# Infini-AI-Lab/Sequoia

Measured on NVIDIA H100. Metric: decoded tokens/sec (mean accepted len/step in config.accepted_tokens_per_step), Sequoia tree speculative decoding, 68m->7B Llama (config c2 unless --config says otherwise), higher is better.
Workload: dtype f16

## Files before the change

sequoia_b200/csrc/sq_gemm.cu:

```cuda
#include <cstdio>
#include <cstdlib>

#include "sq_common.cuh"
#include "sq_ptx.cuh"

struct sq_gemm_plan {
  CUtensorMap tm_a, tm_w;
  __half* c;
  int ldc, n_max, N, K, bn, split, stages, mc, pdl, tiled, epi, n_out;
  int* err_flag;
};

namespace sq {

struct GemmArgs {
  __half* c;
  int ldc, n, N, K, kb_per_split;
  int tiled, kb_total;
  int m0;
  int epi, n_out;
  int* err_flag;
};

constexpr int G_BK = 64;
constexpr int G_THREADS = 384;
constexpr int G_CONSUMER_WARPS = 8;

template <int BN, int STAGES, int SPLIT>
struct GemmSmem {
  static constexpr int A_BYTES = 128 * 128;
  static constexpr int W_BYTES = BN * 128;
  static constexpr int STAGE_BYTES = A_BYTES + ((W_BYTES + 1023) / 1024) * 1024;
  static constexpr int OFF_BAR = STAGES * STAGE_BYTES;
  static constexpr int OFF_RED = OFF_BAR + 256;
  static constexpr int R_STRIDE = BN + 4;
  static constexpr int RED_BYTES = SPLIT > 1 ? 128 * R_STRIDE * 4 : 0;
  static constexpr int TOTAL = OFF_RED + RED_BYTES;
};

__device__ __forceinline__ void tma_load_2d_mc(uint32_t dst, const CUtensorMap* tm, uint32_t bar, int c0, int c1, uint16_t mask) {
  asm volatile(
      "cp.async.bulk.tensor.2d.shared::cluster.global.mbarrier::complete_tx::bytes.multicast::cluster [%0], [%1, {%4, %5}], [%2], %3;" ::"r"(dst),
      "l"(tm), "r"(bar), "h"(mask), "r"(c0), "r"(c1)
      : "memory");
}

template <int BN, int STAGES, int SPLIT, int MC>
__global__ void __launch_bounds__(G_THREADS, 1)
    gemm_tn_kernel(const __grid_constant__ CUtensorMap tm_a, const __grid_constant__ CUtensorMap tm_w, GemmArgs g) {
  using SM = GemmSmem<BN, STAGES, SPLIT>;
  constexpr int NCH = BN / 64;
  extern __shared__ __align__(1024) uint8_t smem_raw[];
  uint8_t* smem = smem_raw + ((1024u - (ptx::smem_u32(smem_raw) & 1023u)) & 1023u);
  const int tid = threadIdx.x, warp = tid >> 5, lane = tid & 31;
  const int n0 = blockIdx.x * BN;
  const int ks = blockIdx.y;
  const int mcr = (MC > 1) ? (int)(blockIdx.x % MC) : 0;
  const int kb0 = ks * g.kb_per_split;
  const int nkb = g.kb_per_split;
  const uint32_t s_base = ptx::smem_u32(smem);
  const uint32_t bar_full = s_base + SM::OFF_BAR, bar_empty = bar_full + 8 * STAGES;

  if (tid == 0) {
#pragma unroll
    for (int s = 0; s < STAGES; ++s) {
      ptx::mbar_init(bar_full + 8 * s, 1);
      ptx::mbar_init(bar_empty + 8 * s, G_CONSUMER_WARPS * MC);
    }
    ptx::fence_barrier_init();
  }
  __syncthreads();
  if (MC > 1)
    asm volatile("barrier.cluster.arrive.release.aligned;\n\tbarrier.cluster.wait.acquire.aligned;" ::: "memory");

  if (warp < 4) {
    if (tid == 0) {
      asm volatile("griddepcontrol.launch_dependents;" ::: "memory");
      const int pre = nkb < STAGES ? nkb : STAGES;
      for (int kb = 0; kb < pre; ++kb) {
        const uint32_t sa = s_base + kb * SM::STAGE_BYTES, sw = sa + SM::A_BYTES;
        ptx::mbar_expect_tx(bar_full + 8 * kb, SM::A_BYTES + SM::W_BYTES);
        if (g.tiled) ptx::tma_load_2d(sw, &tm_w, bar_full + 8 * kb, 0, ((int)blockIdx.x * g.kb_total + kb0 + kb) * BN);
        else ptx::tma_load_2d(sw, &tm_w, bar_full + 8 * kb, (kb0 + kb) * G_BK, n0);
      }
      asm volatile("griddepcontrol.wait;" ::: "memory");
      int stage = 0;
      uint32_t phase = 0;
      for (int kb = 0; kb < nkb; ++kb) {
        const uint32_t sa = s_base + stage * SM::STAGE_BYTES, sw = sa + SM::A_BYTES;
        if (kb >= pre) {
          ptx::mbar_wait_one(bar_empty + 8 * stage, phase ^ 1, g.err_flag, 11);
          ptx::mbar_expect_tx(bar_full + 8 * stage, SM::A_BYTES + SM::W_BYTES);
          if (g.tiled) ptx::tma_load_2d(sw, &tm_w, bar_full + 8 * stage, 0, ((int)blockIdx.x * g.kb_total + kb0 + kb) * BN);
          else ptx::tma_load_2d(sw, &tm_w, bar_full + 8 * stage, (kb0 + kb) * G_BK, n0);
        }
        if (MC == 1) ptx::tma_load_2d(sa, &tm_a, bar_full + 8 * stage, (kb0 + kb) * G_BK, g.m0);
        else tma_load_2d_mc(sa + mcr * (SM::A_BYTES / MC), &tm_a, bar_full + 8 * stage, (kb0 + kb) * G_BK, g.m0 + mcr * (128 / MC),
                            (uint16_t)(((1u << MC) - 1u) << (MC * ks)));
        if (++stage == STAGES) { stage = 0; phase ^= 1; }
      }
    }
  } else {
    const int wg = (warp >> 2) - 1;
    float acc[NCH][32];
#pragma unroll
    for (int c = 0; c < NCH; ++c)
#pragma unroll
      for (int e = 0; e < 32; ++e) acc[c][e] = 0.f;
    auto release = [&](int s) {
      if (lane == 0) {
        if (MC == 1) asm volatile("mbarrier.arrive.shared::cta.b64 _, [%0];" ::"r"(bar_empty + 8 * s) : "memory");
        else
          for (int r = 0; r < MC; ++r) ptx::mbar_arrive_cluster(bar_empty + 8 * s, (uint32_t)(MC * ks + r));
      }
    };
    int stage = 0, prev = -1;
    uint32_t phase = 0;
    for (int kb = 0; kb < nkb; ++kb) {
      ptx::mbar_wait(bar_full + 8 * stage, phase, g.err_flag, 12);
      const uint32_t sa = s_base + stage * SM::STAGE_BYTES + wg * 8192, sw = s_base + stage * SM::STAGE_BYTES + SM::A_BYTES;
      ptx::wgmma_fence();
#pragma unroll
      for (int k = 0; k < G_BK / 16; ++k)
#pragma unroll
        for (int c = 0; c < NCH; ++c)
          ptx::wgmma_ss<0>(acc[c], gmma_desc(sa + k * 32, 16, 1024), gmma_desc(sw + c * 8192 + k * 32, 16, 1024), 1);
      ptx::wgmma_commit();
      asm volatile("wgmma.wait_group.sync.aligned 1;" ::: "memory");
      if (prev >= 0) release(prev);
      prev = stage;
      if (++stage == STAGES) { stage = 0; phase ^= 1; }
    }
    ptx::wgmma_wait_all();
    if (prev >= 0) release(prev);
    const int rbase = wg * 64 + (warp & 3) * 16 + (lane >> 2), q2 = 2 * (lane & 3);
    if (SPLIT == 1 && g.epi == 1) {
#pragma unroll
      for (int h = 0; h < 2; ++h) {
        const int row = rbase + 8 * h;
        if (row >= g.n) continue;
        __half* orow = g.c + (int64_t)(g.m0 + row) * g.ldc;
#pragma unroll
        for (int c = 0; c < NCH; ++c)
#pragma unroll
          for (int j = 0; j < 8; ++j) {
            if ((j & 3) >= 2) continue;
            const int ob = (n0 + c * 64 + (j >> 2) * 32) / 2;
            if (ob >= g.n_out) continue;
            __half o[2];
#pragma unroll
            for (int e = 0; e < 2; ++e) {
              const float x = h2f(f2h(acc[c][4 * j + 2 * h + e]));
              const __half act = f2h(x / (1.0f + expf(-x)));
              o[e] = f2h(h2f(act) * h2f(f2h(acc[c][4 * (j + 2) + 2 * h + e])));
            }
            *reinterpret_cast<__half2*>(orow + ob + (j & 3) * 8 + q2) = __halves2half2(o[0], o[1]);
          }
      }
    } else if (SPLIT == 1) {
#pragma unroll
      for (int h = 0; h < 2; ++h) {
        const int row = rbase + 8 * h;
        if (row >= g.n) continue;
        __half* crow = g.c + (int64_t)(g.m0 + row) * g.ldc + n0;
#pragma unroll
        for (int c = 0; c < NCH; ++c)
#pragma unroll
          for (int j = 0; j < 8; ++j)
            if (n0 + c * 64 + j * 8 < g.N)
              *reinterpret_cast<__half2*>(crow + c * 64 + j * 8 + q2) =
                  __floats2half2_rn(acc[c][4 * j + 2 * h], acc[c][4 * j + 2 * h + 1]);
      }
    } else {
      constexpr int RPC = 128 / SPLIT;
#pragma unroll
      for (int h = 0; h < 2; ++h) {
        const int row = rbase + 8 * h;
        uint32_t dst;
        asm volatile("mapa.shared::cluster.u32 %0, %1, %2;" : "=r"(dst) : "r"(s_base + SM::OFF_RED), "r"((uint32_t)mcr + MC * (row / RPC)));
        dst += (uint32_t)((ks * RPC + row % RPC) * SM::R_STRIDE * 4);
#pragma unroll
        for (int c = 0; c < NCH; ++c)
#pragma unroll
          for (int j = 0; j < 8; ++j)
            asm volatile("st.shared::cluster.v2.f32 [%0], {%1, %2};" ::"r"(dst + (c * 64 + j * 8 + q2) * 4),
                         "f"(acc[c][4 * j + 2 * h]), "f"(acc[c][4 * j + 2 * h + 1])
                         : "memory");
      }
    }
  }
  __syncthreads();

  if (MC > 1 || SPLIT > 1)
    asm volatile("barrier.cluster.arrive.release.aligned;\n\tbarrier.cluster.wait.acquire.aligned;" ::: "memory");

  if (SPLIT > 1) {
    constexpr int RPC = 128 / SPLIT;
    constexpr int CPR = BN / 4;
    const float* red = reinterpret_cast<const float*>(smem + SM::OFF_RED);
    for (int i = tid; i < RPC * CPR; i += G_THREADS) {
      const int lr = i / CPR, cc = i % CPR;
      const int row = ks * RPC + lr;
      if (row >= g.n) continue;
      float4 acc = make_float4(0.f, 0.f, 0.f, 0.f);
#pragma unroll
      for (int s = 0; s < SPLIT; ++s) {
        const float4 o = *reinterpret_cast<const float4*>(red + (s * RPC + lr) * SM::R_STRIDE + cc * 4);
        acc.x += o.x; acc.y += o.y; acc.z += o.z; acc.w += o.w;
      }
      const __half2 lo = __floats2half2_rn(acc.x, acc.y), hi = __floats2half2_rn(acc.z, acc.w);
      uint2 pk;
      pk.x = *reinterpret_cast<const uint32_t*>(&lo);
      pk.y = *reinterpret_cast<const uint32_t*>(&hi);
      *reinterpret_cast<uint2*>(g.c + (int64_t)(g.m0 + row) * g.ldc + n0 + cc * 4) = pk;
    }
  }
}

}

using namespace sq;

typedef CUresult (*PFN_tmapEncodeTiledG)(CUtensorMap*, CUtensorMapDataType, cuuint32_t, void*, const cuuint64_t*,
                                         const cuuint64_t*, const cuuint32_t*, const cuuint32_t*, CUtensorMapInterleave,
                                         CUtensorMapSwizzle, CUtensorMapL2promotion, CUtensorMapFloatOOBfill);

static int encode_2d(CUtensorMap* tm, const void* base, uint64_t inner, uint64_t outer, uint64_t pitch_bytes,
                     uint32_t box_inner, uint32_t box_outer, CUtensorMapL2promotion prom) {
  static PFN_tmapEncodeTiledG fn = nullptr;
  if (!fn) {
    void* p = nullptr;
    cudaDriverEntryPointQueryResult qres;
    if (cudaGetDriverEntryPoint("cuTensorMapEncodeTiled", &p, cudaEnableDefault, &qres) == cudaSuccess &&
        qres == cudaDriverEntryPointSuccess)
      fn = (PFN_tmapEncodeTiledG)p;
  }
  if (!fn) { set_error("cuTensorMapEncodeTiled unavailable"); return SQ_ERR_CUDA; }
  cuuint64_t dims[2] = {inner, outer};
  cuuint64_t strides[1] = {pitch_bytes};
  cuuint32_t box[2] = {box_inner, box_outer};
  cuuint32_t estr[2] = {1, 1};
  CUresult r = fn(tm, CU_TENSOR_MAP_DATA_TYPE_FLOAT16, 2, const_cast<void*>(base), dims, strides, box, estr,
                  CU_TENSOR_MAP_INTERLEAVE_NONE, CU_TENSOR_MAP_SWIZZLE_128B, prom, CU_TENSOR_MAP_FLOAT_OOB_FILL_NONE);
  if (r != CUDA_SUCCESS) { set_error("cuTensorMapEncodeTiled failed: %d", (int)r); return SQ_ERR_CUDA; }
  return SQ_OK;
}

static int sm_count() {
  static int n_sm = 0;
  if (!n_sm) {
    int dev = 0;
    if (cudaGetDevice(&dev) != cudaSuccess || cudaDeviceGetAttribute(&n_sm, cudaDevAttrMultiProcessorCount, dev) != cudaSuccess ||
        n_sm <= 0) {
      cudaGetLastError();
      n_sm = 132;
    }
  }
  return n_sm;
}

static void choose_tiles(sq_gemm_plan* p, bool allow_split) {
  const int N = p->N, kb = p->K / 64;
  const int n_sm = sm_count();
  const int cands[] = {256, 192, 128, 64};
  int best_bn = 128, best_split = 1, best_mc = 1;
  double best_score = -1.0;
  for (int bn : cands) {
    const int tiles = (N + bn - 1) / bn;
    for (int split : {1, 2, 4}) {
      if (kb % split || (split > 1 && !allow_split)) continue;
      if (split > 1 && (bn > 128 || N % bn)) continue;
      const int ctas = tiles * split;
      if (ctas > n_sm) continue;
      for (int mc : {1, 2}) {
        if (mc == 2 && tiles % 2) continue;
        const double a_share = 128.0 / mc, share = bn / (bn + a_share);
        double score = ctas * share;
        if (split > 1) score *= 0.85;
        if (score > best_score) { best_score = score; best_bn = bn; best_split = split; best_mc = mc; }
      }
    }
  }
  p->bn = best_bn; p->split = best_split; p->mc = best_mc;
}

static void pick_tiles(sq_gemm_plan* p) {
  const int kb = p->K / 64;
  const bool allow_split = p->epi == 0;
  choose_tiles(p, allow_split);
  const char* force = getenv("SQ_GEMM_FORCE");
  if (force) {
    int fb = 0, fs = 0, fm = 1;
    const int nf = sscanf(force, "%d,%d,%d", &fb, &fs, &fm);
    const bool bn_ok = fb == 64 || fb == 128 || fb == 192 || fb == 256;
    if (nf >= 2 && bn_ok && (fs == 1 || fs == 2 || fs == 4) && kb % fs == 0 && (fm == 1 || fm == 2) &&
        !(fs > 1 && (fb > 128 || p->N % fb || !allow_split)) && !(fm == 2 && ((p->N + fb - 1) / fb) % 2)) {
      p->bn = fb; p->split = fs; p->mc = fm;
    }
  }
}

extern "C" int sq_gemm_pick_tiles(int N, int K, int* bn, int* split, int* mc) { return sq_gemm_pick_tiles_ex(N, K, 0, bn, split, mc); }

extern "C" int sq_gemm_pick_tiles_ex(int N, int K, int flags, int* bn, int* split, int* mc) {
  SQ_CHECK_ARG(K % 64 == 0 && N % 32 == 0, "sq_gemm_pick_tiles: K %% 64, N %% 32");
  sq_gemm_plan p{};
  p.N = N; p.K = K; p.epi = (flags & SQ_GEMM_SWIGLU) ? 1 : 0;
  pick_tiles(&p);
  *bn = p.bn; *split = p.split; *mc = p.mc;
  return SQ_OK;
}

static int plan_create(sq_gemm_plan** plan, const sq_half* a, int lda, int n_max, const sq_half* w, int N, int K, sq_half* c,
                       int ldc, int* err_flag, int flags);

extern "C" int sq_gemm_plan_create(sq_gemm_plan** plan, const sq_half* a, int lda, int n_max, const sq_half* w, int N,
                                   int K, sq_half* c, int ldc, int* err_flag) {
  return plan_create(plan, a, lda, n_max, w, N, K, c, ldc, err_flag, 0);
}

extern "C" int sq_gemm_plan_create_tiled(sq_gemm_plan** plan, const sq_half* a, int lda, int n_max, const sq_half* w_tiled,
                                         int N, int K, sq_half* c, int ldc, int* err_flag) {
  return plan_create(plan, a, lda, n_max, w_tiled, N, K, c, ldc, err_flag, SQ_GEMM_TILED);
}

extern "C" int sq_gemm_plan_create_ex(sq_gemm_plan** plan, const sq_half* a, int lda, int n_max, const sq_half* w, int N,
                                      int K, sq_half* c, int ldc, int* err_flag, int flags) {
  return plan_create(plan, a, lda, n_max, w, N, K, c, ldc, err_flag, flags);
}

static int plan_create(sq_gemm_plan** plan, const sq_half* a, int lda, int n_max, const sq_half* w, int N, int K, sq_half* c,
                       int ldc, int* err_flag, int flags) {
  const int tiled = (flags & SQ_GEMM_TILED) ? 1 : 0;
  SQ_CHECK_ARG(plan && a && w && c, "sq_gemm_plan_create: null pointer");
  SQ_CHECK_ARG(K % 64 == 0 && N % 32 == 0 && lda % 8 == 0 && ldc % 8 == 0, "sq_gemm_plan_create: K %% 64, N %% 32");
  sq_gemm_plan* p = new sq_gemm_plan();
  p->c = (__half*)c; p->ldc = ldc; p->n_max = n_max; p->N = N; p->K = K; p->err_flag = err_flag;
  p->tiled = tiled; p->epi = (flags & SQ_GEMM_SWIGLU) ? 1 : 0; p->n_out = p->epi ? N / 2 : 0;
  if (p->epi) SQ_CHECK_ARG(N % 32 == 0, "sq_gemm_plan_create: SwiGLU needs N %% 32 == 0");
  pick_tiles(p);
  {
    p->pdl = pdl_enabled() ? 1 : 0;
  }
  p->stages = p->split > 1 ? 4 : (p->bn == 256 ? 4 : p->bn == 192 ? 5 : p->bn == 128 ? 6 : 8);
  int rc = encode_2d(&p->tm_a, a, (uint64_t)K, (uint64_t)n_max, (uint64_t)lda * 2, 64, (uint32_t)(128 / p->mc),
                     CU_TENSOR_MAP_L2_PROMOTION_L2_128B);
  if (!rc) {
    if (tiled) rc = encode_2d(&p->tm_w, w, 64, (uint64_t)((N + p->bn - 1) / p->bn) * (uint64_t)(K / 64) * (uint64_t)p->bn, 128, 64,
                              (uint32_t)p->bn, CU_TENSOR_MAP_L2_PROMOTION_L2_256B);
    else rc = encode_2d(&p->tm_w, w, (uint64_t)K, (uint64_t)N, (uint64_t)K * 2, 64, (uint32_t)p->bn, CU_TENSOR_MAP_L2_PROMOTION_L2_256B);
  }
  if (rc) { delete p; return rc; }
  *plan = p;
  return SQ_OK;
}

extern "C" int sq_gemm_plan_destroy(sq_gemm_plan* plan) {
  delete plan;
  return SQ_OK;
}

template <int BN, int STAGES, int SPLIT, int MC>
static int launch_gemm(sq_gemm_plan* p, GemmArgs& g, cudaStream_t st) {
  using SM = GemmSmem<BN, STAGES, SPLIT>;
  constexpr int smem = SM::TOTAL + 1024;
  static_assert(smem <= 227 * 1024, "shared memory budget");
  static bool attr = false;
  if (!attr) {
    cudaError_t e = cudaFuncSetAttribute(gemm_tn_kernel<BN, STAGES, SPLIT, MC>, cudaFuncAttributeMaxDynamicSharedMemorySize, smem);
    if (e != cudaSuccess) { set_error("sq_gemm: smem attr: %s", cudaGetErrorString(e)); return SQ_ERR_CUDA; }
    attr = true;
  }
  cudaLaunchConfig_t cfg{};
  cfg.gridDim = dim3((p->N + BN - 1) / BN, SPLIT, 1);
  cfg.blockDim = dim3(G_THREADS);
  cfg.dynamicSmemBytes = smem;
  cfg.stream = st;
  cudaLaunchAttribute at[2];
  at[0].id = cudaLaunchAttributeClusterDimension;
  at[0].val.clusterDim.x = MC;
  at[0].val.clusterDim.y = SPLIT;
  at[0].val.clusterDim.z = 1;
  cfg.attrs = at;
  cfg.numAttrs = 1;
  if (p->pdl) {
    at[1].id = cudaLaunchAttributeProgrammaticStreamSerialization;
    at[1].val.programmaticStreamSerializationAllowed = 1;
    cfg.numAttrs = 2;
  }
  cudaError_t e = cudaLaunchKernelEx(&cfg, gemm_tn_kernel<BN, STAGES, SPLIT, MC>, p->tm_a, p->tm_w, g);
  if (e != cudaSuccess) { set_error("sq_gemm: launch failed: %s", cudaGetErrorString(e)); return SQ_ERR_CUDA; }
  SQ_CHECK_LAUNCH("sq_gemm");
  return SQ_OK;
}

static int run_tile(sq_gemm_plan* plan, GemmArgs& g, cudaStream_t st) {
  const int bn = plan->bn, sp = plan->split, mc = plan->mc;
#define SQ_G(BN_, ST_, SP_, MC_) if (bn == BN_ && sp == SP_ && mc == MC_) return launch_gemm<BN_, ST_, SP_, MC_>(plan, g, st)
  SQ_G(256, 4, 1, 1); SQ_G(256, 4, 1, 2);
  SQ_G(192, 5, 1, 1); SQ_G(192, 5, 1, 2);
  SQ_G(128, 6, 1, 1); SQ_G(128, 6, 1, 2); SQ_G(128, 4, 2, 1); SQ_G(128, 4, 4, 1); SQ_G(128, 4, 2, 2); SQ_G(128, 4, 4, 2);
  SQ_G(64, 8, 1, 1); SQ_G(64, 8, 1, 2); SQ_G(64, 4, 2, 1); SQ_G(64, 4, 4, 1); SQ_G(64, 4, 2, 2); SQ_G(64, 4, 4, 2);
#undef SQ_G
  set_error("sq_gemm_run: no kernel for bn=%d split=%d mc=%d", bn, sp, mc);
  return SQ_ERR_UNSUPPORTED;
}

extern "C" int sq_gemm_run(sq_gemm_plan* plan, int n, void* stream) { return sq_gemm_run_at(plan, n, 0, nullptr, 0, stream); }

extern "C" int sq_gemm_run_at(sq_gemm_plan* plan, int n, int a_row0, sq_half* c, int ldc, void* stream) {
  SQ_CHECK_ARG(plan != nullptr, "sq_gemm_run: null plan");
  SQ_CHECK_ARG(n >= 0 && a_row0 >= 0 && a_row0 + n <= plan->n_max, "sq_gemm_run: rows [%d, %d) exceed the plan's n_max=%d", a_row0, a_row0 + n, plan->n_max);
  SQ_CHECK_ARG(c == nullptr || (ldc % 8 == 0 && ((uintptr_t)c % 16) == 0), "sq_gemm_run: output override must be 16 B aligned, pitch %% 8");
  for (int m0 = 0; m0 < n; m0 += 128) {
    GemmArgs g;
    g.n = n - m0 < 128 ? n - m0 : 128; g.N = plan->N; g.K = plan->K;
    g.kb_per_split = plan->K / 64 / plan->split;
    g.tiled = plan->tiled; g.kb_total = plan->K / 64;
    g.m0 = a_row0 + m0; g.epi = plan->epi; g.n_out = plan->n_out;
    if (c) { g.ldc = ldc; g.c = (__half*)c - (int64_t)a_row0 * ldc; }
    else { g.ldc = plan->ldc; g.c = plan->c; }
    g.err_flag = plan->err_flag;
    const int rc = run_tile(plan, g, (cudaStream_t)stream);
    if (rc != SQ_OK) return rc;
  }
  return SQ_OK;
}

extern "C" int sq_gemm_plan_set_epilogue(sq_gemm_plan* plan, int kind, int n_out) {
  SQ_CHECK_ARG(plan != nullptr && (kind == 0 || kind == 1), "sq_gemm_plan_set_epilogue: bad arguments");
  SQ_CHECK_ARG(kind == 0 || (plan->split == 1 && n_out % 16 == 0 && 2 * n_out <= plan->N + 31), "sq_gemm_plan_set_epilogue: SwiGLU needs split 1, n_out %% 16 == 0");
  plan->epi = kind; plan->n_out = n_out;
  return SQ_OK;
}

extern "C" int sq_gemm_plan_info(sq_gemm_plan* plan, int* bn, int* split, int* stages) {
  *bn = plan->bn; *split = plan->split; *stages = plan->stages + 100 * plan->mc;
  return SQ_OK;
}
```

sequoia_b200/model.py:

```python
from __future__ import annotations

import json
import math
import os
from dataclasses import dataclass
from typing import Dict, Optional

import torch

from . import ops

F16 = torch.float16


@dataclass
class LlamaConfigLite:
    hidden_size: int
    intermediate_size: int
    num_hidden_layers: int
    num_attention_heads: int
    num_key_value_heads: int
    vocab_size: int = 32000
    rms_norm_eps: float = 1e-6
    rope_theta: float = 10000.0
    max_position_embeddings: int = 2048
    rope_scaling: Optional[dict] = None

    @property
    def head_dim(self):
        return self.hidden_size // self.num_attention_heads


NAMED_CONFIGS = {
    "llama-68m": LlamaConfigLite(768, 3072, 2, 12, 12),
    "llama-160m": LlamaConfigLite(768, 3072, 12, 12, 12),
    "llama-2-7b": LlamaConfigLite(4096, 11008, 32, 32, 32, rms_norm_eps=1e-5, max_position_embeddings=4096),
    "llama-2-13b": LlamaConfigLite(5120, 13824, 40, 40, 40, rms_norm_eps=1e-5, max_position_embeddings=4096),
    "llama-2-70b": LlamaConfigLite(8192, 28672, 80, 64, 8, rms_norm_eps=1e-5, max_position_embeddings=4096),
    "llama-2-70b-8l": LlamaConfigLite(8192, 28672, 8, 64, 8, rms_norm_eps=1e-5, max_position_embeddings=4096),
    "llama-3.2-1b": LlamaConfigLite(2048, 8192, 16, 32, 8, vocab_size=128256, rms_norm_eps=1e-5, rope_theta=500000.0,
                                    max_position_embeddings=131072,
                                    rope_scaling=dict(rope_type="llama3", factor=32.0, low_freq_factor=1.0,
                                                      high_freq_factor=4.0, original_max_position_embeddings=8192)),
    "llama-3.1-8b": LlamaConfigLite(4096, 14336, 32, 32, 8, vocab_size=128256, rms_norm_eps=1e-5, rope_theta=500000.0,
                                    max_position_embeddings=131072,
                                    rope_scaling=dict(rope_type="llama3", factor=8.0, low_freq_factor=1.0,
                                                      high_freq_factor=4.0, original_max_position_embeddings=8192)),
}


def parse_rope_scaling(rs) -> Optional[dict]:
    if rs is None:
        return None
    kind = rs.get("rope_type", rs.get("type"))
    if kind in (None, "default"):
        return None
    if kind != "llama3":
        raise ValueError(f"rope_scaling type {kind!r} is not supported (supported: None, 'llama3')")
    return dict(rope_type="llama3", factor=float(rs["factor"]), low_freq_factor=float(rs["low_freq_factor"]),
                high_freq_factor=float(rs["high_freq_factor"]),
                original_max_position_embeddings=int(rs["original_max_position_embeddings"]))


def llama3_inv_freq(inv_freq: torch.Tensor, rs: dict) -> torch.Tensor:
    factor, lo, hi = rs["factor"], rs["low_freq_factor"], rs["high_freq_factor"]
    old = rs["original_max_position_embeddings"]
    wavelen = 2 * math.pi / inv_freq
    out = torch.where(wavelen > old / lo, inv_freq / factor, inv_freq)
    smooth = (old / wavelen - lo) / (hi - lo)
    smoothed = (1 - smooth) * out / factor + smooth * out
    medium = ~(wavelen < old / hi) & ~(wavelen > old / lo)
    return torch.where(medium, smoothed, out)


def config_from(obj) -> LlamaConfigLite:
    if isinstance(obj, LlamaConfigLite):
        return obj
    g = (lambda k, d=None: obj.get(k, d)) if isinstance(obj, dict) else (lambda k, d=None: getattr(obj, k, d))
    rp = g("rope_parameters", None) or {}
    theta = g("rope_theta", None) or rp.get("rope_theta")
    rs = g("rope_scaling", None) or (rp or None)
    return LlamaConfigLite(
        hidden_size=g("hidden_size"), intermediate_size=g("intermediate_size"),
        num_hidden_layers=g("num_hidden_layers"), num_attention_heads=g("num_attention_heads"),
        num_key_value_heads=g("num_key_value_heads") or g("num_attention_heads"), vocab_size=g("vocab_size", 32000),
        rms_norm_eps=g("rms_norm_eps", 1e-6), rope_theta=float(theta) if theta else 10000.0,
        max_position_embeddings=g("max_position_embeddings", 2048), rope_scaling=parse_rope_scaling(rs))


def _load_state_dict_dir(path: str) -> Dict[str, torch.Tensor]:
    sd: Dict[str, torch.Tensor] = {}
    files = sorted(os.listdir(path))
    st = [f for f in files if f.endswith(".safetensors")]
    if st:
        from safetensors.torch import load_file
        for f in st:
            sd.update(load_file(os.path.join(path, f)))
        return sd
    for f in files:
        if (f.startswith("pytorch_model") and f.endswith(".bin")) or (f.startswith("model") and f.endswith(".pt")):
            sd.update(torch.load(os.path.join(path, f), map_location="cpu"))
    if not sd:
        raise FileNotFoundError(f"no weight files (*.safetensors / *.bin) in {path}")
    return sd


class _RandomInit:

    def __init__(self, cfg: LlamaConfigLite, seed: int, device):
        self.cfg, self.device = cfg, device
        self.g = torch.Generator(device=device)
        self.g.manual_seed(seed)

    def get(self, name: str, shape) -> torch.Tensor:
        if name.endswith("norm.weight") or "layernorm" in name:
            return torch.ones(shape, dtype=F16, device=self.device)
        t = torch.empty(shape, dtype=F16, device=self.device)
        t.normal_(0.0, 0.02, generator=self.g)
        return t


class _DictSource:
    def __init__(self, sd: Dict[str, torch.Tensor], device):
        self.sd, self.device = sd, device

    def get(self, name: str, shape) -> torch.Tensor:
        if name == "lm_head.weight" and name not in self.sd:
            name = "model.embed_tokens.weight"
        t = self.sd[name]
        assert tuple(t.shape) == tuple(shape), (name, t.shape, shape)
        return t.to(device=self.device, dtype=F16)


def resolve_model(model_name_or_path, device):
    if isinstance(model_name_or_path, dict):
        cfg = config_from(model_name_or_path["config"])
        return cfg, _DictSource(model_name_or_path["state_dict"], device)
    s = str(model_name_or_path)
    if s.startswith("random-init:"):
        parts = s.split(":")
        cfg = NAMED_CONFIGS[parts[1].lower()]
        seed = int(parts[2]) if len(parts) > 2 else 0
        return cfg, _RandomInit(cfg, seed, device)
    if os.path.isdir(s):
        with open(os.path.join(s, "config.json")) as f:
            cfg = config_from(json.load(f))
        return cfg, _DictSource(_load_state_dict_dir(s), device)
    raise FileNotFoundError(
        f"{s!r}: expected a local model directory or 'random-init:<{'|'.join(NAMED_CONFIGS)}>[:seed]' "
        "(there is no network access for hub downloads)")


def rope_cache(cfg: LlamaConfigLite, max_length: int, device):
    d = cfg.head_dim
    inv_freq = 1.0 / (cfg.rope_theta ** (torch.arange(0, d, 2, dtype=torch.float32) / d))
    if cfg.rope_scaling is not None:
        inv_freq = llama3_inv_freq(inv_freq, parse_rope_scaling(cfg.rope_scaling))
    t = torch.arange(max(cfg.max_position_embeddings, max_length), dtype=torch.float32)
    freqs = torch.outer(t, inv_freq)
    emb = torch.cat((freqs, freqs), dim=-1)
    return (emb.cos()[:max_length].to(F16).to(device).contiguous(), emb.sin()[:max_length].to(F16).to(device).contiguous())


class TPInfo:
    def __init__(self, group=None):
        import torch.distributed as dist
        self.group = group
        if group is None:
            self.rank, self.size = 0, 1
        else:
            self.rank, self.size = dist.get_rank(group), dist.get_world_size(group)

    def all_reduce(self, t: torch.Tensor):
        if self.size > 1:
            import torch.distributed as dist
            dist.all_reduce(t, group=self.group)


def full_state_dict(cfg: LlamaConfigLite, src) -> Dict[str, torch.Tensor]:
    h, D, V = cfg.hidden_size, cfg.head_dim, cfg.vocab_size
    Hf, Hkvf, If = cfg.num_attention_heads, cfg.num_key_value_heads, cfg.intermediate_size
    sd = {"model.embed_tokens.weight": src.get("model.embed_tokens.weight", (V, h))}
    for l in range(cfg.num_hidden_layers):
        p = f"model.layers.{l}."
        for name, shape in (("self_attn.q_proj.weight", (Hf * D, h)), ("self_attn.k_proj.weight", (Hkvf * D, h)),
                            ("self_attn.v_proj.weight", (Hkvf * D, h)), ("self_attn.o_proj.weight", (h, Hf * D)),
                            ("mlp.gate_proj.weight", (If, h)), ("mlp.up_proj.weight", (If, h)),
                            ("mlp.down_proj.weight", (h, If)), ("input_layernorm.weight", (h,)),
                            ("post_attention_layernorm.weight", (h,))):
            sd[p + name] = src.get(p + name, shape)
    sd["model.norm.weight"] = src.get("model.norm.weight", (h,))
    sd["lm_head.weight"] = src.get("lm_head.weight", (V, h))
    return sd


def load_sharded_weights(cfg: LlamaConfigLite, src, rank: int, tp: int) -> dict:
    h, D, V = cfg.hidden_size, cfg.head_dim, cfg.vocab_size
    Hf, Hkvf, If = cfg.num_attention_heads, cfg.num_key_value_heads, cfg.intermediate_size
    assert Hf % tp == 0 and Hkvf % tp == 0 and If % tp == 0, "heads / FFN width must divide the TP degree"
    H, Hkv, I, r = Hf // tp, Hkvf // tp, If // tp, rank
    out = {"embed": src.get("model.embed_tokens.weight", (V, h)), "layers": []}
    for l in range(cfg.num_hidden_layers):
        p = f"model.layers.{l}."
        wq = src.get(p + "self_attn.q_proj.weight", (Hf * D, h))[r * H * D:(r + 1) * H * D]
        wk = src.get(p + "self_attn.k_proj.weight", (Hkvf * D, h))[r * Hkv * D:(r + 1) * Hkv * D]
        wv = src.get(p + "self_attn.v_proj.weight", (Hkvf * D, h))[r * Hkv * D:(r + 1) * Hkv * D]
        wo = src.get(p + "self_attn.o_proj.weight", (h, Hf * D))[:, r * H * D:(r + 1) * H * D]
        wg = src.get(p + "mlp.gate_proj.weight", (If, h))[r * I:(r + 1) * I]
        wu = src.get(p + "mlp.up_proj.weight", (If, h))[r * I:(r + 1) * I]
        wd = src.get(p + "mlp.down_proj.weight", (h, If))[:, r * I:(r + 1) * I]
        out["layers"].append(dict(
            wqkv=torch.cat([wq, wk, wv], dim=0).contiguous(), wo=wo.contiguous(),
            wgu=torch.cat([wg, wu], dim=0).contiguous(), wd=wd.contiguous(),
            ln1=src.get(p + "input_layernorm.weight", (h,)), ln2=src.get(p + "post_attention_layernorm.weight", (h,))))
        del wq, wk, wv, wo, wg, wu, wd
    out["norm"] = src.get("model.norm.weight", (h,))
    out["lm_head"] = src.get("lm_head.weight", (V, h))
    return out


class LlamaRunner:

    PROJECTIONS = ("wqkv", "wo", "wgu", "wd")

    def __init__(self, model_name_or_path, max_length: int, device="cuda:0", tp_group=None, n_max: Optional[int] = None,
                 batch_size: int = 1, weight_format: str = "fp16"):
        if weight_format not in ("fp16", "fp8"):
            raise ValueError(f"weight_format must be 'fp16' or 'fp8', got {weight_format!r}")
        if weight_format == "fp8" and tp_group is not None:
            raise NotImplementedError("FP8 target weights run on one GPU: tensor parallelism needs weight_format='fp16'")
        self.weight_format = weight_format
        self.device = torch.device(device)
        self.B = batch_size
        self.cfg, src = resolve_model(model_name_or_path, self.device)
        cfg = self.cfg
        self.tp = TPInfo(tp_group)
        tp, r = self.tp.size, self.tp.rank
        assert cfg.num_attention_heads % tp == 0 and cfg.num_key_value_heads % tp == 0 and cfg.intermediate_size % tp == 0
        self.M = max_length
        self.n_max = n_max or max_length * batch_size
        self.H, self.Hkv, self.D = cfg.num_attention_heads // tp, cfg.num_key_value_heads // tp, cfg.head_dim
        self.I = cfg.intermediate_size // tp
        h, D, V = cfg.hidden_size, self.D, cfg.vocab_size
        self.h, self.V, self.L = h, V, cfg.num_hidden_layers
        if weight_format == "fp8":
            shapes = (((self.H + 2 * self.Hkv) * D, h), (h, self.H * D), (2 * self.I, h), (h, self.I))
            if any(n % 64 or k % 64 for n, k in shapes):
                raise ValueError(f"weight_format='fp8' needs every layer projection (N, K) to be multiples of 64, got {shapes}")
        wts = load_sharded_weights(cfg, src, r, tp)
        self.embed, self.layers, self.norm, self.lm_head = wts["embed"], wts["layers"], wts["norm"], wts["lm_head"]
        self.cos, self.sin = rope_cache(cfg, max_length, self.device)
        self.eps = float(cfg.rms_norm_eps)
        n = self.n_max
        dev = self.device
        z = lambda *s: torch.zeros(*s, dtype=F16, device=dev)
        self.hidden, self.normed = z(n, h), z(n, h)
        self.qkv = z(n, (self.H + 2 * self.Hkv) * D)
        self.attn_out, self.proj = z(n, self.H * D), z(n, h)
        self.gate_up, self.act = z(n, 2 * self.I), z(n, self.I)
        self.logits = z(n, V)
        self.k_cache = torch.zeros(self.L, batch_size, self.Hkv, max_length, D, dtype=F16, device=dev)
        self.v_cache = torch.zeros_like(self.k_cache)
        self.plan = ops.AttnPlan(self.qkv, n, self.H, self.Hkv, D, self.k_cache, self.v_cache, self.attn_out)
        self.gemm_err = torch.zeros(4, dtype=torch.int32, device=dev)
        self.lm_plan = None
        if weight_format == "fp8":
            io = dict(wqkv=(self.normed, self.qkv), wo=(self.attn_out, self.proj), wgu=(self.normed, self.gate_up),
                      wd=(self.act, self.proj))
            for ly in self.layers:
                for k in self.PROJECTIONS:
                    q, s = ops.quantize_fp8(ly.pop(k))
                    ly[k + "_fp8"] = ops.GemmFp8Plan(io[k][0], q, s, io[k][1], self.gemm_err)
                    del q
            torch.cuda.empty_cache()
        stream_sized = h >= 2048
        ok = stream_sized and tp == 1 and weight_format == "fp16" and self.I % 16 == 0 and h % 64 == 0
        self.gu_interleaved = False
        if ok and ops.gemm_pick_tiles(2 * self.I, h, ops.GEMM_SWIGLU)[2] == 1:
            self.gu_interleaved = True
            for ly in self.layers:
                ly["wgu"] = ops.interleave_gate_up(ly["wgu"][:self.I], ly["wgu"][self.I:])
                ly["wgu_plan"] = ops.GemmPlan(self.normed, ly["wgu"], self.act, self.gemm_err, swiglu=True)
        if stream_sized and V % 32 == 0 and h % 64 == 0:
            self.lm_plan = ops.GemmPlan(self.normed, self.lm_head, self.logits, self.gemm_err)
        self.draft_plan = None
        if (os.environ.get("SQ_DRAFT_ATTN", "1") != "0" and tp == 1 and batch_size == 1 and
                ops.draft_supported(h, self.H, self.Hkv, D, max_length)):
            self.draft_plan = ops.DraftPlan(h, self.L, self.H, max_length, self.k_cache, self.v_cache)
        self.peer = None
        if self.tp.size > 1 and os.environ.get("SQ_TP_MODE", "fused") == "fused":
            from .peer import PeerBuffers
            self.peer = PeerBuffers(tp_group, self.device, n, h)

    def _gate_up_act(self, ly, n: int):
        plan = ly.get("wgu_plan")
        if plan is not None and 96 < n <= 128:
            plan.run(n)
            return
        self._project(ly, "wgu", self.normed, n, self.gate_up)
        ops.silu_mul(self.gate_up, self.act, n, interleaved=self.gu_interleaved)

    def _project(self, ly, k: str, a: torch.Tensor, n: int, out: torch.Tensor):
        plan = ly.get(k + "_fp8")
        if plan is not None:
            plan.run(n)
        else:
            torch.mm(a[:n], ly[k].t(), out=out[:n])

    def weight_bytes(self) -> int:
        b = 2 * (self.embed.numel() + self.lm_head.numel() + self.norm.numel())
        for ly in self.layers:
            b += 2 * (ly["ln1"].numel() + ly["ln2"].numel())
            b += sum(ly[k + "_fp8"].weight_bytes() if k + "_fp8" in ly else 2 * ly[k].numel() for k in self.PROJECTIONS)
        return b

    @torch.no_grad()
    def forward(self, n: int, tokens: torch.Tensor, position_ids: torch.Tensor, storage_ids: torch.Tensor, *,
                state=None, n0: int = 0, kv_end: int = 0, prefix_len: int = 0, dense_mask=None, mask_ld: int = 0,
                tree_bits=None, tree_words: int = 0, tree_size: int = 0, logits_out: Optional[torch.Tensor] = None,
                logits_from: int = 0, skip_lm_head: bool = False, batch: bool = False,
                logits_to: Optional[int] = None) -> Optional[torch.Tensor]:
        B = self.B if batch else 1
        N = n * B
        assert 0 < N <= self.n_max
        assert not batch or (state is not None and dense_mask is None)
        H, Hkv, D, M = self.H, self.Hkv, self.D, self.M
        small = (not batch and self.draft_plan is not None and state is not None and n <= ops.DraftPlan.MAX_ROWS
                 and dense_mask is None)
        if batch:
            ops.embed_rows_batch(self.embed, tokens, n, self.hidden, state, n0=n0)
        else:
            ops.embed_rows(self.embed, tokens, n, self.hidden, state=state, n0=n0)
        n_seq = n

        def attend(l):
            if batch:
                ops.rope_kv_append_batch(self.qkv, H, Hkv, D, self.cos, self.sin, position_ids, storage_ids, n_seq,
                                         self.k_cache[l], self.v_cache[l], M, state, n0=n0)
                ops.tree_attn_batch(self.plan, l, n_seq, state=state, n0=n0, kv_end=kv_end, tree_bits=tree_bits,
                                    tree_words=tree_words, tree_size=tree_size)
                return
            ops.rope_kv_append(self.qkv, H, Hkv, D, self.cos, self.sin, position_ids, storage_ids, n, self.k_cache[l],
                               self.v_cache[l], M, state=state, n0=n0)
            if small:
                self.draft_plan.attention(l, n, self.qkv, self.attn_out, state, n0, kv_end, tree_bits, tree_words,
                                          tree_size)
            else:
                ops.tree_attn(self.plan, l, n, state=state, n0=n0, kv_end=kv_end, prefix_len=prefix_len,
                              dense_mask=dense_mask, mask_ld=mask_ld, tree_bits=tree_bits, tree_words=tree_words,
                              tree_size=tree_size)

        self._layers(N, attend)
        if skip_lm_head:
            return None
        return self._lm_head(logits_from, N if logits_to is None else logits_to, logits_out)

    @torch.no_grad()
    def forward_ragged(self, parts, tokens: torch.Tensor, position_ids: torch.Tensor, storage_ids: torch.Tensor, *,
                       state: torch.Tensor, tree_bits=None, tree_words: int = 0, tree_size: int = 0) -> None:
        if self.tp.size > 1:
            raise NotImplementedError("forward_ragged runs on one GPU: tensor-parallel engines use forward(batch=True)")
        geo = [tuple(int(x) for x in p[:4]) for p in parts]
        row0, _ = ops.ragged_layout(geo, self.B, self.n_max)
        for (seq, n, _, _), (*_, m, out) in zip(geo, parts):
            if not 0 < m <= n or out is None or tuple(out.shape) != (m, self.V):
                raise ValueError(f"sequence {seq}: {m} logit rows of {n} into {None if out is None else tuple(out.shape)}")
        H, Hkv, D, M = self.H, self.Hkv, self.D, self.M
        arr = ops.ragged_parts(geo)
        ops.embed_rows_ragged(self.embed, tokens, arr, self.hidden, state)

        def attend(l):
            ops.rope_kv_append_ragged(self.qkv, H, Hkv, D, self.cos, self.sin, position_ids, storage_ids, arr,
                                      self.k_cache[l], self.v_cache[l], M, state)
            ops.tree_attn_ragged(self.plan, l, arr, state=state, tree_bits=tree_bits, tree_words=tree_words,
                                 tree_size=tree_size)

        self._layers(row0[-1], attend)
        for (_, n, _, _), (*_, m, out), r0 in zip(geo, parts, row0):
            self._lm_head(r0 + n - m, r0 + n, out)

    def _layers(self, n: int, attend):
        ops.rmsnorm(self.hidden, self.layers[0]["ln1"], self.normed, n, self.eps)
        for l, ly in enumerate(self.layers):
            self._project(ly, "wqkv", self.normed, n, self.qkv)
            attend(l)
            nxt = self.layers[l + 1]["ln1"] if l + 1 < self.L else self.norm
            if self.peer is not None:
                torch.mm(self.attn_out[:n], ly["wo"].t(), out=self.peer.buf[0][:n])
                self.peer.allreduce_add_rmsnorm(0, self.hidden, ly["ln2"], self.normed, n, self.eps)
                self._gate_up_act(ly, n)
                torch.mm(self.act[:n], ly["wd"].t(), out=self.peer.buf[1][:n])
                self.peer.allreduce_add_rmsnorm(1, self.hidden, nxt, self.normed, n, self.eps)
                continue
            self._project(ly, "wo", self.attn_out, n, self.proj)
            self.tp.all_reduce(self.proj[:n])
            ops.add_rmsnorm(self.hidden, self.proj, ly["ln2"], self.normed, n, self.eps)
            self._gate_up_act(ly, n)
            self._project(ly, "wd", self.act, n, self.proj)
            self.tp.all_reduce(self.proj[:n])
            ops.add_rmsnorm(self.hidden, self.proj, nxt, self.normed, n, self.eps)

    def _lm_head(self, start: int, end: int, out: Optional[torch.Tensor]) -> torch.Tensor:
        m = end - start
        out = out if out is not None else self.logits[:m]
        if self.lm_plan is not None and m <= 128 and out.stride(-1) == 1 and out.stride(0) % 8 == 0 and out.data_ptr() % 16 == 0:
            self.lm_plan.run(m, a_row0=start, out=out)
        else:
            torch.mm(self.normed[start:end], self.lm_head.t(), out=out)
        return out
```

Measured before the change: 188.1.

## Route verify projections through custom split-K GEMM with wide-tile splits and cost model

Adds custom TMA/WGMMA GEMM plans for the qkv, o and down projections of the 7B target, used when the verify batch holds 97-128 tokens instead of torch.mm. The GEMM kernel now supports uneven K splits, split-K for 192/256-wide tiles up to split 8, and reuses the pipeline ring buffer as the split-K reduction scratch after a cluster barrier. Tile selection moves to a bandwidth-based latency model. The aim is better SM coverage on small-M weight-bound GEMMs; the risk is reduction overhead, the extra cluster barrier, and a worse choice than cuBLAS for some shapes.

```diff
diff --git a/sequoia_b200/csrc/sq_gemm.cu b/sequoia_b200/csrc/sq_gemm.cu
--- a/sequoia_b200/csrc/sq_gemm.cu
+++ b/sequoia_b200/csrc/sq_gemm.cu
@@ -15,7 +15,7 @@
 
 struct GemmArgs {
   __half* c;
-  int ldc, n, N, K, kb_per_split;
+  int ldc, n, N, K;
   int tiled, kb_total;
   int m0;
   int epi, n_out;
@@ -32,10 +32,9 @@
   static constexpr int W_BYTES = BN * 128;
   static constexpr int STAGE_BYTES = A_BYTES + ((W_BYTES + 1023) / 1024) * 1024;
   static constexpr int OFF_BAR = STAGES * STAGE_BYTES;
-  static constexpr int OFF_RED = OFF_BAR + 256;
+  static constexpr int TOTAL = OFF_BAR + 256;
   static constexpr int R_STRIDE = BN + 4;
-  static constexpr int RED_BYTES = SPLIT > 1 ? 128 * R_STRIDE * 4 : 0;
-  static constexpr int TOTAL = OFF_RED + RED_BYTES;
+  static_assert(SPLIT == 1 || 128 * R_STRIDE * 4 <= OFF_BAR, "split-K reduction buffer must fit in the ring");
 };
 
 __device__ __forceinline__ void tma_load_2d_mc(uint32_t dst, const CUtensorMap* tm, uint32_t bar, int c0, int c1, uint16_t mask) {
@@ -56,8 +55,8 @@
   const int n0 = blockIdx.x * BN;
   const int ks = blockIdx.y;
   const int mcr = (MC > 1) ? (int)(blockIdx.x % MC) : 0;
-  const int kb0 = ks * g.kb_per_split;
-  const int nkb = g.kb_per_split;
+  const int kb0 = ks * g.kb_total / SPLIT;
+  const int nkb = (ks + 1) * g.kb_total / SPLIT - kb0;
   const uint32_t s_base = ptx::smem_u32(smem);
   const uint32_t bar_full = s_base + SM::OFF_BAR, bar_empty = bar_full + 8 * STAGES;
 
@@ -73,6 +72,9 @@
   if (MC > 1)
     asm volatile("barrier.cluster.arrive.release.aligned;\n\tbarrier.cluster.wait.acquire.aligned;" ::: "memory");
 
+  float acc[NCH][32];
+  const int wg = (warp >> 2) - 1;
+  const int rbase = wg * 64 + (warp & 3) * 16 + (lane >> 2), q2 = 2 * (lane & 3);
   if (warp < 4) {
     if (tid == 0) {
       asm volatile("griddepcontrol.launch_dependents;" ::: "memory");
@@ -100,9 +102,8 @@
         if (++stage == STAGES) { stage = 0; phase ^= 1; }
       }
     }
+    __syncwarp();
   } else {
-    const int wg = (warp >> 2) - 1;
-    float acc[NCH][32];
 #pragma unroll
     for (int c = 0; c < NCH; ++c)
 #pragma unroll
@@ -133,51 +134,17 @@
     }
     ptx::wgmma_wait_all();
     if (prev >= 0) release(prev);
-    const int rbase = wg * 64 + (warp & 3) * 16 + (lane >> 2), q2 = 2 * (lane & 3);
-    if (SPLIT == 1 && g.epi == 1) {
-#pragma unroll
-      for (int h = 0; h < 2; ++h) {
-        const int row = rbase + 8 * h;
-        if (row >= g.n) continue;
-        __half* orow = g.c + (int64_t)(g.m0 + row) * g.ldc;
-#pragma unroll
-        for (int c = 0; c < NCH; ++c)
-#pragma unroll
-          for (int j = 0; j < 8; ++j) {
-            if ((j & 3) >= 2) continue;
-            const int ob = (n0 + c * 64 + (j >> 2) * 32) / 2;
-            if (ob >= g.n_out) continue;
-            __half o[2];
-#pragma unroll
-            for (int e = 0; e < 2; ++e) {
-              const float x = h2f(f2h(acc[c][4 * j + 2 * h + e]));
-              const __half act = f2h(x / (1.0f + expf(-x)));
-              o[e] = f2h(h2f(act) * h2f(f2h(acc[c][4 * (j + 2) + 2 * h + e])));
-            }
-            *reinterpret_cast<__half2*>(orow + ob + (j & 3) * 8 + q2) = __halves2half2(o[0], o[1]);
-          }
-      }
-    } else if (SPLIT == 1) {
-#pragma unroll
-      for (int h = 0; h < 2; ++h) {
-        const int row = rbase + 8 * h;
-        if (row >= g.n) continue;
-        __half* crow = g.c + (int64_t)(g.m0 + row) * g.ldc + n0;
-#pragma unroll
-        for (int c = 0; c < NCH; ++c)
-#pragma unroll
-          for (int j = 0; j < 8; ++j)
-            if (n0 + c * 64 + j * 8 < g.N)
-              *reinterpret_cast<__half2*>(crow + c * 64 + j * 8 + q2) =
-                  __floats2half2_rn(acc[c][4 * j + 2 * h], acc[c][4 * j + 2 * h + 1]);
-      }
-    } else {
+  }
+
+  if (SPLIT > 1) {
+    asm volatile("barrier.cluster.arrive.release.aligned;\n\tbarrier.cluster.wait.acquire.aligned;" ::: "memory");
+    if (warp >= 4) {
       constexpr int RPC = 128 / SPLIT;
 #pragma unroll
       for (int h = 0; h < 2; ++h) {
         const int row = rbase + 8 * h;
         uint32_t dst;
-        asm volatile("mapa.shared::cluster.u32 %0, %1, %2;" : "=r"(dst) : "r"(s_base + SM::OFF_RED), "r"((uint32_t)mcr + MC * (row / RPC)));
+        asm volatile("mapa.shared::cluster.u32 %0, %1, %2;" : "=r"(dst) : "r"(s_base), "r"((uint32_t)mcr + MC * (row / RPC)));
         dst += (uint32_t)((ks * RPC + row % RPC) * SM::R_STRIDE * 4);
 #pragma unroll
         for (int c = 0; c < NCH; ++c)
@@ -188,6 +155,43 @@
                          : "memory");
       }
     }
+  } else if (warp >= 4 && g.epi == 1) {
+#pragma unroll
+    for (int h = 0; h < 2; ++h) {
+      const int row = rbase + 8 * h;
+      if (row >= g.n) continue;
+      __half* orow = g.c + (int64_t)(g.m0 + row) * g.ldc;
+#pragma unroll
+      for (int c = 0; c < NCH; ++c)
+#pragma unroll
+        for (int j = 0; j < 8; ++j) {
+          if ((j & 3) >= 2) continue;
+          const int ob = (n0 + c * 64 + (j >> 2) * 32) / 2;
+          if (ob >= g.n_out) continue;
+          __half o[2];
+#pragma unroll
+          for (int e = 0; e < 2; ++e) {
+            const float x = h2f(f2h(acc[c][4 * j + 2 * h + e]));
+            const __half act = f2h(x / (1.0f + expf(-x)));
+            o[e] = f2h(h2f(act) * h2f(f2h(acc[c][4 * (j + 2) + 2 * h + e])));
+          }
+          *reinterpret_cast<__half2*>(orow + ob + (j & 3) * 8 + q2) = __halves2half2(o[0], o[1]);
+        }
+    }
+  } else if (warp >= 4) {
+#pragma unroll
+    for (int h = 0; h < 2; ++h) {
+      const int row = rbase + 8 * h;
+      if (row >= g.n) continue;
+      __half* crow = g.c + (int64_t)(g.m0 + row) * g.ldc + n0;
+#pragma unroll
+      for (int c = 0; c < NCH; ++c)
+#pragma unroll
+        for (int j = 0; j < 8; ++j)
+          if (n0 + c * 64 + j * 8 < g.N)
+            *reinterpret_cast<__half2*>(crow + c * 64 + j * 8 + q2) =
+                __floats2half2_rn(acc[c][4 * j + 2 * h], acc[c][4 * j + 2 * h + 1]);
+    }
   }
   __syncthreads();
 
@@ -197,11 +201,11 @@
   if (SPLIT > 1) {
     constexpr int RPC = 128 / SPLIT;
     constexpr int CPR = BN / 4;
-    const float* red = reinterpret_cast<const float*>(smem + SM::OFF_RED);
+    const float* red = reinterpret_cast<const float*>(smem);
     for (int i = tid; i < RPC * CPR; i += G_THREADS) {
       const int lr = i / CPR, cc = i % CPR;
       const int row = ks * RPC + lr;
-      if (row >= g.n) continue;
+      if (row >= g.n || n0 + cc * 4 >= g.N) continue;
       float4 acc = make_float4(0.f, 0.f, 0.f, 0.f);
 #pragma unroll
       for (int s = 0; s < SPLIT; ++s) {
@@ -259,44 +263,50 @@
   return n_sm;
 }
 
+static int tile_stages(int bn, int split, int mc) {
+  const int ring = bn == 256 ? 4 : bn == 192 ? 5 : bn == 128 ? 6 : bn == 64 ? 8 : 0;
+  if (!ring || (mc != 1 && mc != 2)) return 0;
+  if (split == 1) return ring;
+  if (bn <= 128) return (split == 2 || split == 4) ? 4 : 0;
+  return (mc == 1 && (split == 2 || split == 4 || split == 8)) ? ring : 0;
+}
+
+static bool tile_legal(const sq_gemm_plan* p, int bn, int split, int mc, bool allow_split) {
+  return tile_stages(bn, split, mc) && split <= p->K / 64 && (split == 1 || allow_split) &&
+         !(mc == 2 && ((p->N + bn - 1) / bn) % 2);
+}
+
 static void choose_tiles(sq_gemm_plan* p, bool allow_split) {
-  const int N = p->N, kb = p->K / 64;
+  const double kHbmGBs = 2650.0, kSmGBsPer192KB = 50.0, kFixedUs = 2.0, kRedUsPerCol = 1.0 / 96;
+  const int N = p->N, K = p->K;
   const int n_sm = sm_count();
-  const int cands[] = {256, 192, 128, 64};
-  int best_bn = 128, best_split = 1, best_mc = 1;
-  double best_score = -1.0;
-  for (int bn : cands) {
+  int best_bn = 128, best_split = 1;
+  double best_us = 1e30, best_ring = 0.0;
+  for (int bn : {256, 192, 128, 64}) {
     const int tiles = (N + bn - 1) / bn;
-    for (int split : {1, 2, 4}) {
-      if (kb % split || (split > 1 && !allow_split)) continue;
-      if (split > 1 && (bn > 128 || N % bn)) continue;
-      const int ctas = tiles * split;
-      if (ctas > n_sm) continue;
-      for (int mc : {1, 2}) {
-        if (mc == 2 && tiles % 2) continue;
-        const double a_share = 128.0 / mc, share = bn / (bn + a_share);
-        double score = ctas * share;
-        if (split > 1) score *= 0.85;
-        if (score > best_score) { best_score = score; best_bn = bn; best_split = split; best_mc = mc; }
-      }
-    }
-  }
-  p->bn = best_bn; p->split = best_split; p->mc = best_mc;
+    for (int split : {1, 2, 4, 8}) {
+      if (!tile_legal(p, bn, split, 1, allow_split) || tiles * split > n_sm) continue;
+      const double ring_kb = tile_stages(bn, split, 1) * (16.0 + (bn * 128 + 1023) / 1024);
+      const double w_gb = (double)tiles * bn * K * 2 / 1e9, cta_gb = (double)(bn + 128) * K / split * 2 / 1e9;
+      double us = fmax(w_gb / kHbmGBs, cta_gb / (kSmGBsPer192KB * ring_kb / 192.0)) * 1e6 + kFixedUs;
+      if (split > 1) us += kRedUsPerCol * bn * split;
+      const bool tie = us < 1.02 * best_us && (split < best_split || (split == best_split && ring_kb > best_ring));
+      if (us < 0.98 * best_us || tie) {
+        best_us = us; best_ring = ring_kb; best_bn = bn; best_split = split;
+      }
+    }
+  }
+  p->bn = best_bn; p->split = best_split; p->mc = 1;
 }
 
 static void pick_tiles(sq_gemm_plan* p) {
-  const int kb = p->K / 64;
   const bool allow_split = p->epi == 0;
   choose_tiles(p, allow_split);
   const char* force = getenv("SQ_GEMM_FORCE");
   if (force) {
     int fb = 0, fs = 0, fm = 1;
     const int nf = sscanf(force, "%d,%d,%d", &fb, &fs, &fm);
-    const bool bn_ok = fb == 64 || fb == 128 || fb == 192 || fb == 256;
-    if (nf >= 2 && bn_ok && (fs == 1 || fs == 2 || fs == 4) && kb % fs == 0 && (fm == 1 || fm == 2) &&
-        !(fs > 1 && (fb > 128 || p->N % fb || !allow_split)) && !(fm == 2 && ((p->N + fb - 1) / fb) % 2)) {
-      p->bn = fb; p->split = fs; p->mc = fm;
-    }
+    if (nf >= 2 && tile_legal(p, fb, fs, fm, allow_split)) { p->bn = fb; p->split = fs; p->mc = fm; }
   }
 }
 
@@ -342,7 +352,7 @@
   {
     p->pdl = pdl_enabled() ? 1 : 0;
   }
-  p->stages = p->split > 1 ? 4 : (p->bn == 256 ? 4 : p->bn == 192 ? 5 : p->bn == 128 ? 6 : 8);
+  p->stages = tile_stages(p->bn, p->split, p->mc);
   int rc = encode_2d(&p->tm_a, a, (uint64_t)K, (uint64_t)n_max, (uint64_t)lda * 2, 64, (uint32_t)(128 / p->mc),
                      CU_TENSOR_MAP_L2_PROMOTION_L2_128B);
   if (!rc) {
@@ -363,7 +373,7 @@
 template <int BN, int STAGES, int SPLIT, int MC>
 static int launch_gemm(sq_gemm_plan* p, GemmArgs& g, cudaStream_t st) {
   using SM = GemmSmem<BN, STAGES, SPLIT>;
-  constexpr int smem = SM::TOTAL + 1024;
+  constexpr int smem = SM::TOTAL + 1024 > 116 * 1024 ? SM::TOTAL + 1024 : 116 * 1024;
   static_assert(smem <= 227 * 1024, "shared memory budget");
   static bool attr = false;
   if (!attr) {
@@ -394,6 +404,16 @@
   return SQ_OK;
 }
 
+static int run_tile_wide_split(sq_gemm_plan* plan, GemmArgs& g, cudaStream_t st) {
+  const int bn = plan->bn, sp = plan->split, mc = plan->mc;
+#define SQ_GW(BN_, ST_, SP_, MC_) if (bn == BN_ && sp == SP_ && mc == MC_) return launch_gemm<BN_, ST_, SP_, MC_>(plan, g, st)
+  SQ_GW(256, 4, 2, 1); SQ_GW(256, 4, 4, 1); SQ_GW(256, 4, 8, 1);
+  SQ_GW(192, 5, 2, 1); SQ_GW(192, 5, 4, 1); SQ_GW(192, 5, 8, 1);
+#undef SQ_GW
+  set_error("sq_gemm_run: no kernel for bn=%d split=%d mc=%d", bn, sp, mc);
+  return SQ_ERR_UNSUPPORTED;
+}
+
 static int run_tile(sq_gemm_plan* plan, GemmArgs& g, cudaStream_t st) {
   const int bn = plan->bn, sp = plan->split, mc = plan->mc;
 #define SQ_G(BN_, ST_, SP_, MC_) if (bn == BN_ && sp == SP_ && mc == MC_) return launch_gemm<BN_, ST_, SP_, MC_>(plan, g, st)
@@ -402,8 +422,7 @@
   SQ_G(128, 6, 1, 1); SQ_G(128, 6, 1, 2); SQ_G(128, 4, 2, 1); SQ_G(128, 4, 4, 1); SQ_G(128, 4, 2, 2); SQ_G(128, 4, 4, 2);
   SQ_G(64, 8, 1, 1); SQ_G(64, 8, 1, 2); SQ_G(64, 4, 2, 1); SQ_G(64, 4, 4, 1); SQ_G(64, 4, 2, 2); SQ_G(64, 4, 4, 2);
 #undef SQ_G
-  set_error("sq_gemm_run: no kernel for bn=%d split=%d mc=%d", bn, sp, mc);
-  return SQ_ERR_UNSUPPORTED;
+  return run_tile_wide_split(plan, g, st);
 }
 
 extern "C" int sq_gemm_run(sq_gemm_plan* plan, int n, void* stream) { return sq_gemm_run_at(plan, n, 0, nullptr, 0, stream); }
@@ -415,7 +434,6 @@
   for (int m0 = 0; m0 < n; m0 += 128) {
     GemmArgs g;
     g.n = n - m0 < 128 ? n - m0 : 128; g.N = plan->N; g.K = plan->K;
-    g.kb_per_split = plan->K / 64 / plan->split;
     g.tiled = plan->tiled; g.kb_total = plan->K / 64;
     g.m0 = a_row0 + m0; g.epi = plan->epi; g.n_out = plan->n_out;
     if (c) { g.ldc = ldc; g.c = (__half*)c - (int64_t)a_row0 * ldc; }
diff --git a/sequoia_b200/model.py b/sequoia_b200/model.py
--- a/sequoia_b200/model.py
+++ b/sequoia_b200/model.py
@@ -222,6 +222,7 @@
 class LlamaRunner:
 
     PROJECTIONS = ("wqkv", "wo", "wgu", "wd")
+    VERIFY_PLANS = ("wqkv", "wo", "wd")
 
     def __init__(self, model_name_or_path, max_length: int, device="cuda:0", tp_group=None, n_max: Optional[int] = None,
                  batch_size: int = 1, weight_format: str = "fp16"):
@@ -281,6 +282,11 @@
             for ly in self.layers:
                 ly["wgu"] = ops.interleave_gate_up(ly["wgu"][:self.I], ly["wgu"][self.I:])
                 ly["wgu_plan"] = ops.GemmPlan(self.normed, ly["wgu"], self.act, self.gemm_err, swiglu=True)
+        if ok and self.I % 64 == 0 and (self.H * D) % 64 == 0:
+            io = dict(wqkv=(self.normed, self.qkv), wo=(self.attn_out, self.proj), wd=(self.act, self.proj))
+            for ly in self.layers:
+                for k in self.VERIFY_PLANS:
+                    ly[k + "_plan"] = ops.GemmPlan(io[k][0], ly[k], io[k][1], self.gemm_err)
         if stream_sized and V % 32 == 0 and h % 64 == 0:
             self.lm_plan = ops.GemmPlan(self.normed, self.lm_head, self.logits, self.gemm_err)
         self.draft_plan = None
@@ -302,6 +308,8 @@
 
     def _project(self, ly, k: str, a: torch.Tensor, n: int, out: torch.Tensor):
         plan = ly.get(k + "_fp8")
+        if plan is None and 96 < n <= 128:
+            plan = ly.get(k + "_plan")
         if plan is not None:
             plan.run(n)
         else:
```

New measurement: 183.3, median of 6. 2.6% lower.
